# dvega68/MC33_c_library

Measured on AMD Instinct MI355X. Metric: Mvoxels/s, higher is better.
Workload: dtype f32; 1 GPU; 1024x1024x1024-point float grid cos x+cos y+cos z on h=8/1023, iso=0.0, calculate_isosurface (sweep+scan+emit), grid and outputs resident in HBM; cells=1070599167, sweep=one pass over the grid per isovalue, vertices=3903888, triangles=7795976, parallelism=single GPU

## Files before the change

### mc33_c_library_amd/build.py

```python
import os
import shutil
import subprocess
import sys

PKG = os.path.dirname(os.path.abspath(__file__))
CSRC = os.path.join(PKG, "csrc")
ROOT = os.path.dirname(PKG)
BUILD = os.path.join(PKG, "_build")

HIPCC = os.environ.get("HIPCC") or shutil.which("hipcc") or "/opt/rocm/bin/hipcc"
GCC = os.environ.get("CC") or "gcc"

HIP_FLAGS = ["-O3", "--offload-arch=gfx950", "-ffp-contract=off", "-std=c++17", "-fPIC", "-Wall", "-Wno-unused-function", "-Wno-inline-asm"]
if os.environ.get("MC33_DEV", "0") == "1":
    HIP_FLAGS.append("-DMC33_DEV")
C_FLAGS = ["-O2", "-ffp-contract=off", "-std=c11", "-fPIC", "-Wall", "-Wextra"]

VARIANTS = {
    "f32": {"hip": [], "c": []},
    "u16": {"hip": ["-DMC33_GRD_U16"], "c": ["-DINTEGER_GRD", "-DGRD_TYPE_SIZE=2"]},
    "u8": {"hip": ["-DMC33_GRD_U8"], "c": ["-DINTEGER_GRD", "-DGRD_TYPE_SIZE=1"]},
    "u32": {"hip": ["-DMC33_GRD_U32"], "c": ["-DINTEGER_GRD", "-DGRD_TYPE_SIZE=4"]},
    "f64": {"hip": ["-DMC33_GRD_F64"], "c": ["-DGRD_TYPE_SIZE=8"]},
}


def lib_path(dtype, ortho=False, nneg=False):
    return os.path.join(PKG, "libMC33_%s%s%s.so" % (dtype, "_ortho" if ortho else "", "_nneg" if nneg else ""))


NNEG_TYPES = ("f32", "u16", "u8", "u32", "f64")


def _newer(target, deps):
    if not os.path.exists(target):
        return True
    t = os.path.getmtime(target)
    return any(os.path.getmtime(d) > t for d in deps)


def _run(cmd):
    print("+ " + " ".join(cmd), flush=True)
    subprocess.check_call(cmd)


C_SOURCES = ["mc33_capi.c", "mc33_surface_io.c", "mc33_grid_io.c"]
HIP_HEADERS = ["mc33_cell.h", "mc33_lut_data.h", "mc33_rules_data.h",
               "mc33_sweep_plan.h", "mc33_records.hip.h", "mc33_sweep_pack.h", "mc33_sweep.hip.h", "mc33_tail.hip.h", "mc33_emit.hip.h", "mc33_context.hip.h", "mc33_extract.hip.h",
               "mc33_property.hip.h", "mc33_mesh.hip.h", "mc33_measure.hip.h", "mc33_topology.hip.h", "mc33_filter.hip.h", "mc33_smooth.hip.h", "mc33_cap.hip.h", "mc33_render.hip.h",
               "mc33_distance.hip.h",
               "mc33_simplify.hip.h", "mc33_clip.hip.h", "mc33_section.hip.h", "mc33_resample.hip.h", "mc33_curvature.hip.h",
               "mc33_spectrum.hip.h"]


def build(dtype, force=False, verbose_resources=False):
    os.makedirs(BUILD, exist_ok=True)
    var = VARIANTS[dtype]
    incs = [os.path.join(ROOT, "include", f) for f in ("mc33_hip.h", "marching_cubes_33.h")] + [os.path.abspath(__file__)]
    hip_src = os.path.join(CSRC, "mc33_kernels.hip")
    hip_obj = os.path.join(BUILD, "mc33_kernels_%s.o" % dtype)
    objs, relink = [hip_obj], force
    if force or _newer(hip_obj, [hip_src] + [os.path.join(CSRC, f) for f in HIP_HEADERS] + incs):
        extra = ["-Rpass-analysis=kernel-resource-usage"] if verbose_resources else []
        _run([HIPCC] + HIP_FLAGS + var["hip"] + extra + ["-c", hip_src, "-o", hip_obj])
        relink = True
    for name in C_SOURCES:
        src = os.path.join(CSRC, name)
        obj = os.path.join(BUILD, "%s_%s.o" % (os.path.splitext(name)[0], dtype))
        if force or _newer(obj, [src] + incs):
            _run([GCC] + C_FLAGS + var["c"] + ["-c", src, "-o", obj])
            relink = True
        objs.append(obj)
    out = lib_path(dtype)
    if relink or _newer(out, objs):
        _run([HIPCC, "--offload-arch=gfx950", "-shared", "-fPIC"] + objs + ["-o", out])
    oobjs, relink = [hip_obj], force
    for name in C_SOURCES:
        src = os.path.join(CSRC, name)
        obj = os.path.join(BUILD, "%s_%s_ortho.o" % (os.path.splitext(name)[0], dtype))
        if force or _newer(obj, [src] + incs):
            _run([GCC] + C_FLAGS + var["c"] + ["-DGRD_ORTHOGONAL", "-c", src, "-o", obj])
            relink = True
        oobjs.append(obj)
    oout = lib_path(dtype, ortho=True)
    if relink or _newer(oout, oobjs):
        _run([HIPCC, "--offload-arch=gfx950", "-shared", "-fPIC"] + oobjs + ["-o", oout])
    if dtype in NNEG_TYPES:
        for ortho, base in ((False, objs), (True, oobjs)):
            nobjs, relink = list(base), force
            src = os.path.join(CSRC, "mc33_capi.c")
            obj = os.path.join(BUILD, "mc33_capi_%s%s_nneg.o" % (dtype, "_ortho" if ortho else ""))
            if force or _newer(obj, [src] + incs):
                _run([GCC] + C_FLAGS + var["c"] + (["-DGRD_ORTHOGONAL"] if ortho else []) + ["-DMC33_NORMAL_NEG=1", "-c", src, "-o", obj])
                relink = True
            nobjs[1 + C_SOURCES.index("mc33_capi.c")] = obj
            nout = lib_path(dtype, ortho=ortho, nneg=True)
            if relink or _newer(nout, nobjs):
                _run([HIPCC, "--offload-arch=gfx950", "-shared", "-fPIC"] + nobjs + ["-o", nout])
    return out


def build_all(force=False):
    from concurrent.futures import ThreadPoolExecutor
    with ThreadPoolExecutor(max_workers=min(5, os.cpu_count() or 1)) as ex:
        return list(ex.map(lambda d: build(d, force), VARIANTS))


if __name__ == "__main__":
    build_all(force="--force" in sys.argv)
```

### mc33_c_library_amd/csrc/mc33_kernels.hip

```cpp
#include <hip/hip_runtime.h>

#include <cstdarg>
#include <cstddef>
#include <cstdio>
#include <cstdlib>
#include <cstring>
#include <chrono>
#include <mutex>
#include <algorithm>
#include <cmath>
#include <limits>
#include <thread>
#include <type_traits>
#include <utility>
#include <vector>

#include "../../include/mc33_hip.h"
#ifdef MC33_GRD_F64
#define MC33_REAL_DOUBLE
#endif
#if !defined(MC33_GRD_U8) && !defined(MC33_GRD_U16) && !defined(MC33_GRD_U32)
#define MC33_NAN_SAMPLES 1
#else
#define MC33_INT_SAMPLES 1
#endif
#include "mc33_cell.h"
#include "mc33_lut_data.h"
#include "mc33_rules_data.h"

using namespace mc33;

#if defined(MC33_GRD_U16)
typedef uint16_t sample_t;
#define MC33_SAMPLE_BYTES 2
#elif defined(MC33_GRD_U8)
typedef uint8_t sample_t;
#define MC33_SAMPLE_BYTES 1
#elif defined(MC33_GRD_U32)
typedef uint32_t sample_t;
#define MC33_SAMPLE_BYTES 4
#elif defined(MC33_GRD_F64)
typedef double sample_t;
#define MC33_SAMPLE_BYTES 8
#else
typedef float sample_t;
#define MC33_SAMPLE_BYTES 4
#endif

#include "mc33_sweep_plan.h"
#include "mc33_records.hip.h"
#include "mc33_sweep_pack.h"
#include "mc33_sweep.hip.h"
#include "mc33_tail.hip.h"
#include "mc33_emit.hip.h"
#include "mc33_context.hip.h"
#include "mc33_extract.hip.h"
#include "mc33_property.hip.h"
#include "mc33_mesh.hip.h"
#include "mc33_measure.hip.h"
#include "mc33_topology.hip.h"
#include "mc33_filter.hip.h"
#include "mc33_smooth.hip.h"
#include "mc33_cap.hip.h"
#include "mc33_render.hip.h"
#include "mc33_distance.hip.h"
#include "mc33_simplify.hip.h"
#include "mc33_clip.hip.h"
#include "mc33_section.hip.h"
#include "mc33_resample.hip.h"
#include "mc33_curvature.hip.h"
#include "mc33_spectrum.hip.h"
```

### mc33_c_library_amd/csrc/mc33_sweep.hip.h

```cpp

#if defined(MC33_GRD_U16)
constexpr int SWEEP_PACK = 2;
#elif defined(MC33_GRD_U8)
constexpr int SWEEP_PACK = 4;
#else
constexpr int SWEEP_PACK = 1;
#endif

template <bool V>
__global__ __launch_bounds__(256) void k_ranges(const GridView<sample_t> G, const Params P, const uint32_t nYT, const uint32_t nplanes, RangeEntry *out, RangeEntry *blocks) {
	constexpr uint32_t VS = 16u / (uint32_t)sizeof(sample_t);
	struct alignas(16) Piece { sample_t s[VS]; };
	constexpr real_t INF = std::numeric_limits<real_t>::infinity();
	__shared__ real_t s_col0[4][4][2];
	__shared__ real_t s_blk[4][RANGE_BLOCKS][2];
	const uint32_t lane = threadIdx.x & 63u, nXG = (P.nseg + 3u) / 4u, wv = (uint32_t)__builtin_amdgcn_readfirstlane((int)(threadIdx.x >> 6));
	const uint32_t xg = blockIdx.x % nXG, yt = (blockIdx.x / nXG) % nYT, pl = blockIdx.x / nXG / nYT;
	const uint32_t seg = xg * 4u + wv;
	const bool active = seg < P.nseg && pl < nplanes;
	const uint32_t xbase = seg * SEG_CELLS, y0 = yt * 63u, nrows = min(64u, P.ny + 1u - y0), xlast = min(xbase + SEG_CELLS, P.nx);
	const sample_t *base = G.p + (uint64_t)pl * G.slice + (uint64_t)y0 * G.pitch;
	const bool right = wv < 3u && seg + 1u < P.nseg;
	auto take = [&](real_t &lo, real_t &hi, sample_t s) __attribute__((always_inline)) {
		const real_t f = (real_t)s;
// ... 262 lines not shown
		whole = (e.x & MC33_PACK_GROUP) != 0u;
	}
	if (wtile >= a.ntiles) return;
	const SweepTile tile = a.tiles[wtile];
	const uint32_t yt = tile.yt, seg = tile.seg;
	const Params &P = a.P;
	bool grouped = true;
	if constexpr (R == 2) grouped = whole;
	else {
		const uint32_t t0 = wtile & ~3u;
		if (t0 + 3u >= a.ntiles) grouped = false;
		else {
			const SweepTile first = a.tiles[t0];
#pragma unroll
			for (uint32_t k = 1; k < 4; k++) {
				const SweepTile o = a.tiles[t0 + k];
				grouped = grouped && o.seg == first.seg + k && o.yt == first.yt && o.z_lo == first.z_lo && o.z_hi == first.z_hi;
			}
		}
	}
	const unsigned long long t_start = a.trace ? __builtin_amdgcn_s_memrealtime() : 0ull;
	const unsigned long long c_start = a.trace ? __builtin_amdgcn_s_memtime() : 0ull;
	if (R == 1 && a.ranges) {
		const uint32_t wme = (uint32_t)__builtin_amdgcn_readfirstlane((int)(threadIdx.x >> 6));
		const uint32_t seg0 = grouped ? seg - wme : seg, nk = grouped ? 4u : 1u, me = grouped ? wme : 0u;
		const uint32_t p0r = tile.z_lo == a.P.zs ? tile.z_lo : tile.z_lo + 1u;
		uint32_t m = 0xFFFFFFFFu;
		for (uint32_t p = p0r + lane; p <= tile.z_hi; p += 64u) {
			const RangeEntry *row = a.ranges + (((uint64_t)(p - a.G.z0) * a.sd.nYT + yt) * a.sd.nseg + seg0);
			static_for<4>([&](auto kc) __attribute__((always_inline)) {
				constexpr int k = decltype(kc)::value;
				if ((uint32_t)k < nk) {
					const RangeEntry e = row[k];
					static_for<NI>([&](auto qc) __attribute__((always_inline)) {
						constexpr int q = decltype(qc)::value;
						const real_t v = a.lane[q].iso;
						m &= ~(((e.hi < v ? 0u : 1u) | (e.lo > v ? 0u : 2u)) << (2 * NI * k + 2 * q));
					});
				}
			});
		}
#pragma unroll
		for (int dlt = 32; dlt; dlt >>= 1) m &= (uint32_t)__shfl_xor((int)m, dlt);
		m = (uint32_t)__builtin_amdgcn_readfirstlane((int)m);
		constexpr uint32_t EVEN = NI == 4 ? 0x55u : NI == 2 ? 0x5u : 0x1u, ALLQ = (1u << (2 * NI)) - 1u;
		const uint32_t one_side = (m | m >> 1);
		bool dead_any = false;
		static_for<4>([&](auto kc) __attribute__((always_inline)) {
			constexpr int k = decltype(kc)::value;
			if ((uint32_t)k < nk) dead_any = dead_any || ((one_side >> (2 * NI * k)) & EVEN) == EVEN;
		});
		const uint32_t mine = (m >> (2u * NI * me)) & ALLQ;
		dead_me = ((mine | mine >> 1) & EVEN) == EVEN;
		if (dead_any) grouped = false;
		if (dead_me) {
			if (lane == 0) {
				static_for<NI>([&](auto qc) __attribute__((always_inline)) {
					constexpr int q = decltype(qc)::value;
					const bool above = ((mine >> (2 * q)) & 2u) != 0u;
					const uint32_t hb = above ? 0xFFFFFFFFu : 0u;
					uint4 *h = a.lane[q].edge_hdr + (uint64_t)wtile * 2u * 2u;
					if (p0r != tile.z_lo) { h[0] = uint4{hb, hb, 0u, 0u}; h[1] = uint4{0u, 0u, above ? PLANE_UNIFORM1 : PLANE_UNIFORM0, 0u}; }
					if (tile.z_hi < a.z_end) { h[2] = uint4{hb, hb, 0u, 0u}; h[3] = uint4{0u, 0u, above ? PLANE_UNIFORM1 : PLANE_UNIFORM0, 0u}; }
				});
				if (NI == 1 && a.skipped) atomicAdd(a.skipped + ((mine & 2u) ? 2 : 1), 1u);
			}
		}
	}
	__shared__ uint64_t s_mail[2][4][NI][2];
	const bool from_right = grouped && (uint32_t)__builtin_amdgcn_readfirstlane((int)(threadIdx.x >> 6)) < 3u;
	const uint32_t xbase = seg * SEG_CELLS, y0 = yt * 63u;
	const uint32_t nrows = min(64u, P.ny + 1 - y0);
	const uint32_t z_lo = tile.z_lo, z_hi = tile.z_hi;
	const uint32_t pl0 = z_lo == P.zs ? z_lo : z_lo + 1u;
	const bool has_above = z_hi < a.z_end;

	const uint32_t rowbytes = a.G.pitch * (uint32_t)sizeof(sample_t);
	uint32_t xo[LPR];
#pragma unroll
	for (int k = 0; k < LPR; k++)
		xo[k] = S == 1 ? min(xbase + 64u * k + lane, P.nx) * (uint32_t)sizeof(sample_t)
		               : min(xbase + (256u / LPR) * k + (uint32_t)S * lane, P.nx & ~(uint32_t)(S - 1)) * (uint32_t)sizeof(sample_t);
	uint64_t valid[4];
	{
		uint64_t vstd[4];
		valid_masks(xbase, P.nx, vstd);
		from_standard<S>(vstd, valid);
	}
	const bool rowvalid = lane < 63u && y0 + lane < P.ny;
	const uint32_t xh = min(lane, nrows - 1) * rowbytes + min(xbase + SEG_CELLS, P.nx) * (uint32_t)sizeof(sample_t);

	constexpr bool PREV_LDS = NI >= 4;
	__shared__ uint64_t s_prev[PREV_LDS ? NI : 1][4][PREV_LDS ? 256 : 1];
	__shared__ uint64_t s_prevz[PREV_LDS ? NI : 1][2][4];
	__shared__ uint32_t s_prevh[PREV_LDS ? NI : 1][PREV_LDS ? 256 : 1];
	constexpr bool DEFER = NI == 1;
	__shared__ typename std::conditional<DEFER, SweepLog, uint32_t>::type s_log[DEFER ? 4 : 1];
	uint32_t log_np = 0, log_ns = 0, log_edge = LOG_NONE;
	uint32_t pend_chunk[NI];
	unsigned long long pend_sum[NI];
#pragma unroll
	for (int q = 0; q < NI; q++) { pend_chunk[q] = 0u; pend_sum[q] = 0ull; }
	const uint32_t wv = (uint32_t)__builtin_amdgcn_readfirstlane((int)(threadIdx.x >> 6));
	uint64_t cur[NI][4], prev[PREV_LDS ? 1 : NI][4];
	uint64_t c64[NI][4];
	uint32_t cur_h[NI], prev_h[PREV_LDS ? 1 : NI];
	uint64_t cur_zc[NI], prev_zc[PREV_LDS ? 1 : NI], zcacc[NI];
	uint64_t cur_z[NI], prev_z[PREV_LDS ? 1 : NI], zacc[NI];
	constexpr bool ZMIN_REG = !(sizeof(real_t) == 8 && NI >= 4);
	real_t zmin[NI];
	uint64_t zeq[NI];
	bool cur_written[NI], prev_written[NI];
	real_t iso[NI];
#pragma unroll
	for (int q = 0; q < NI; q++) {
#pragma unroll
		for (int k = 0; k < 4; k++) {
			if constexpr (PREV_LDS) s_prev[q][k][threadIdx.x] = 0; else prev[q][k] = 0;
			c64[q][k] = 0;
		}
		cur_h[q] = 0; cur_z[q] = zacc[q] = 0; cur_zc[q] = zcacc[q] = 0;
		if constexpr (PREV_LDS) { s_prevz[q][0][wv] = 0; s_prevz[q][1][wv] = 0; s_prevh[q][threadIdx.x] = 0; } else { prev_z[q] = 0; prev_zc[q] = 0; prev_h[q] = 0; }
		cur_written[q] = prev_written[q] = false; zmin[q] = 1; zeq[q] = 0;
		iso[q] = a.lane[q].iso;
	}

	const uint32_t NB = (nrows + (uint32_t)RB - 1u) / (uint32_t)RB;
	const uint32_t T = dead_me ? 0u : (z_hi - pl0 + 1u) * NB;
	const uint32_t tile_bytes = dead_me ? 0u : nrows * rowbytes;
#ifndef MC33_SWEEP_AUX
#if defined(MC33_GRD_U16) || defined(MC33_GRD_U8)
#define MC33_SWEEP_AUX 0
#else
#define MC33_SWEEP_AUX 2
#endif
#endif
#if defined(MC33_GRD_U16)
#define MC33_LOAD(rs, vo, so) ((float)(uint16_t)__builtin_amdgcn_raw_buffer_load_b16(rs, vo, so, MC33_SWEEP_AUX))
#elif defined(MC33_GRD_U8)
#define MC33_LOAD(rs, vo, so) ((float)(uint8_t)__builtin_amdgcn_raw_buffer_load_b8(rs, vo, so, MC33_SWEEP_AUX))
#elif defined(MC33_GRD_U32)
#define MC33_LOAD(rs, vo, so) ((float)(uint32_t)__builtin_amdgcn_raw_buffer_load_b32(rs, vo, so, MC33_SWEEP_AUX))
#elif defined(MC33_GRD_F64)
#define MC33_LOAD(rs, vo, so) (__builtin_bit_cast(double, __builtin_amdgcn_raw_buffer_load_b64(rs, vo, so, MC33_SWEEP_AUX)))
#else
#define MC33_LOAD(rs, vo, so) (__uint_as_float(__builtin_amdgcn_raw_buffer_load_b32(rs, vo, so, MC33_SWEEP_AUX)))
#endif
	typedef typename std::conditional<S == 1, real_t, uint32_t>::type raw_t;
	constexpr bool BS = BLOCKS;
	static_assert(!BLOCKS || (MC33_BLOCK_SKIP && R == 2 && NI == 1 && S == 1), "blocks are left out by the float single-isovalue sweep with a live list");
	auto block_word = [&](uint32_t p) __attribute__((always_inline)) -> uint64_t {
		if constexpr (BS) {
			if (a.blockw) {
				const unsigned long long w = a.blockw[((uint64_t)(min(p, z_hi) - a.G.z0) * a.sd.nYT + yt) * a.sd.nseg + seg];
				return u64((uint32_t)__builtin_amdgcn_readfirstlane((int)(uint32_t)w), (uint32_t)__builtin_amdgcn_readfirstlane((int)(uint32_t)(w >> 32)));
			}
		}
		return 0ull;
	};
	uint64_t bwi = block_word(pl0), bwi_n = block_word(pl0 + 1u), bwp = bwi, bwp_n = bwi_n;
	auto issue = [&](raw_t (&d)[16], real_t &hv, uint32_t p, uint32_t bi) __attribute__((always_inline)) {
		const sample_t *base = a.G.p + (uint64_t)(p - a.G.z0) * a.G.slice + (uint64_t)y0 * a.G.pitch;
		const __amdgpu_buffer_rsrc_t rs = __builtin_amdgcn_make_buffer_rsrc((void *)base, 0, tile_bytes, 0x00020000);
		const uint32_t r = bi * (uint32_t)RB;
		uint32_t codes = 0u, hcode = 0u;
		if constexpr (BS) { codes = (uint32_t)(bwi >> (8u * (bi >> 2))) & 0xFFu; hcode = (uint32_t)(bwi >> (32u + 2u * (bi >> 2))) & 3u; }
#pragma unroll
		for (int rr = 0; rr < RB; rr++) {
			const uint32_t so = min(r + rr, nrows - 1) * rowbytes;
#pragma unroll
			for (int k = 0; k < LPR; k++) {
				if constexpr (BS) {
					const bool dk = ((codes >> (2 * k)) & 3u) != 0u;
					d[rr * LPR + k] = MC33_LOAD(rs, dk ? 0xFFFFFFF0u : xo[k], dk ? 0u : so);
				} else
				if constexpr (S == 1) d[rr * LPR + k] = MC33_LOAD(rs, xo[k], so);
				else d[rr * LPR + k] = __builtin_amdgcn_raw_buffer_load_b32(rs, xo[k], so, MC33_SWEEP_AUX);
			}
		}
		if constexpr (NI == 1 && sizeof(real_t) == 4) {
			const bool wanted = ((lane / (uint32_t)RB) == bi) & !from_right & !(MC33_DEBUG_BITS(a) & 64u) & (hcode == 0u);
			if (wanted) hv = MC33_LOAD(rs, xh, 0u);
		} else
		hv = MC33_LOAD(rs, ((lane / (uint32_t)RB) == bi && !from_right && !(MC33_DEBUG_BITS(a) & 64u)) ? xh : 0xFFFFFFF0u, 0u);
	};
	auto sample = [&](const raw_t (&dd)[16], int rr, int k) -> real_t {
		if constexpr (S == 1) return dd[rr * 4 + k];
		else if constexpr (S == 2) return (real_t)((dd[rr * 2 + (k >> 1)] >> (16 * (k & 1))) & 0xFFFFu);
		else return (real_t)((dd[rr] >> (8 * k)) & 0xFFu);
	};

	auto raw_sample = [&](const raw_t (&dd)[16], int rr, int k) -> uint32_t {
		if constexpr (S == 2) return ((uint32_t)dd[rr * 2 + (k >> 1)] >> (16 * (k & 1))) & 0xFFFFu;
		else if constexpr (S == 4) return ((uint32_t)dd[rr] >> (8 * k)) & 0xFFu;
		else return 0u;
	};
	auto log_flush = [&]() __attribute__((always_inline)) {
		if constexpr (DEFER) {
			SweepLog &G = s_log[wv];
			const SweepLane &L0 = a.lane[0];
			const uint32_t ln = fresh_lane();
			__builtin_amdgcn_fence(__ATOMIC_ACQ_REL, "wavefront");
			for (uint32_t k = 0; k < log_np; k++) {
				const uint64_t slot = readlane64(G.plane_slot[k], 0);
				__builtin_amdgcn_raw_buffer_store_b32(G.plane[k][ln], record_rsrc(L0.slice_compact + slot * 64u, 256u), ln * 4u, 0u, 0);
				if (ln == 0) L0.plane_fmt[slot] = (uint8_t)PLANE_COMPACT;
			}
			{
				const bool mine = ln < log_ns;
				const uint32_t e = mine ? ln : 0u;
				const uint32_t *w = G.hdr[e];
				const uint64_t slot = G.hdr_slot[e];
				if (mine) {
					uint32_t *h = (uint32_t *)(L0.slice_hdr + slot);
					*(uint4 *)h = uint4{w[0], w[1], w[2], w[3]};
					*(uint4 *)(h + 4) = uint4{w[4], w[5], w[6], w[7]};
					*(uint2 *)(h + 8) = uint2{w[8], w[9]};
				}
				const uint32_t chunk = mine ? (uint32_t)(slot / SLOT_CHUNK) : 0xFFFFFFFFu;
				const uint32_t cells = mine ? w[5] : 0u, batches = mine ? w[10] : 0u;
				uint32_t sum_c = cells, sum_b = batches;
#pragma unroll 1
				for (uint32_t dlt = 1; dlt < log_ns; dlt++) {
					const uint32_t c2 = __shfl_down(chunk, dlt), v2 = __shfl_down(cells, dlt), b2 = __shfl_down(batches, dlt);
					const bool same = c2 == chunk && ln + dlt < 64u;
					sum_c += same ? v2 : 0u; sum_b += same ? b2 : 0u;
				}
				const uint32_t before = __shfl_up(chunk, 1);
				if (mine && (ln == 0u || before != chunk)) atomicAdd(L0.slot_part + chunk, (unsigned long long)sum_b << 32 | sum_c);
			}
			if (log_edge != LOG_NONE) {
				if (log_edge == PLANE_COMPACT) __builtin_amdgcn_raw_buffer_store_b32(G.edge[ln], record_rsrc(L0.edge_bits + (uint64_t)wtile * 2u * 128u, 2048u), ln * 4u, 0u, 0);
				if (ln == 0) {
					const uint32_t *e = G.edge_hdr;
					L0.edge_hdr[(uint64_t)wtile * 2u * 2u] = uint4{e[0], e[1], e[2], e[3]};
					L0.edge_hdr[(uint64_t)wtile * 2u * 2u + 1u] = uint4{e[4], e[5], e[6], e[7]};
				}
			}
			__builtin_amdgcn_fence(__ATOMIC_ACQ_REL, "wavefront");
			log_np = 0; log_ns = 0; log_edge = LOG_NONE;
		}
	};
	auto log_plane = [&](uint64_t slot, const uint64_t (&w)[4], uint32_t ln) __attribute__((always_inline)) {
		if constexpr (DEFER) {
			uint32_t desc;
			if (encode_plane<S>(w, desc)) {
				if (log_np == LOG_PLANES) log_flush();
				SweepLog &G = s_log[wv];
				G.plane[log_np][ln] = desc;
				if (ln == 0) G.plane_slot[log_np] = slot;
				log_np++;
			} else {
				store_plane_raw<S>(a.lane[0].slice_bits + slot * 128u, w, ln);
				if (ln == 0) a.lane[0].plane_fmt[slot] = (uint8_t)PLANE_RAW;
			}
		}
	};
	auto log_header = [&](uint64_t slot, uint64_t bp, uint64_t bc, uint64_t zrows, uint64_t zcols, const uint64_t (&act)[4], uint32_t ln) __attribute__((always_inline)) {
		if constexpr (DEFER) {
			uint32_t ncell = __popcll(act[0]) + __popcll(act[1]) + __popcll(act[2]) + __popcll(act[3]);
#pragma unroll
			for (int dlt = 32; dlt; dlt >>= 1) ncell += __shfl_xor(ncell, dlt);
			if (log_ns == LOG_SLICES) log_flush();
			if (ln == 0) {
				SweepLog &G = s_log[wv];
				uint32_t *w = G.hdr[log_ns];
				w[0] = a.lane[0].epoch << 2 | SLICE_VALID | (zrows ? SLICE_HAS_ISO : 0u);
				w[1] = (uint32_t)bp; w[2] = (uint32_t)(bp >> 32); w[3] = (uint32_t)bc; w[4] = (uint32_t)(bc >> 32); w[5] = ncell;
				w[6] = (uint32_t)zrows; w[7] = (uint32_t)(zrows >> 32); w[8] = (uint32_t)zcols; w[9] = (uint32_t)(zcols >> 32);
				w[10] = (ncell + 63u) >> 6;
				G.hdr_slot[log_ns] = slot;
			}
			log_ns++;
		}
	};
	real_t halo = 0;
	auto process = [&](const raw_t (&dd)[16], const real_t &hv, uint32_t p, uint32_t bi) __attribute__((always_inline)) {
		const uint32_t r = bi * (uint32_t)RB;
		uint32_t codes = 0u;
		if constexpr (BS) {
			constexpr real_t INF = std::numeric_limits<real_t>::infinity();
			codes = (uint32_t)(bwp >> (8u * (bi >> 2))) & 0xFFu;
			const uint32_t hcode = (uint32_t)(bwp >> (32u + 2u * (bi >> 2))) & 3u;
			const real_t hsub = hcode == 1u ? -INF : INF;
			halo = (lane / (uint32_t)RB) == bi ? (hcode ? hsub : hv) : halo;
		} else
		halo = (lane / (uint32_t)RB) == bi ? hv : halo;
		unrolled_for<RB, (S >= 4)>([&](auto rc) __attribute__((always_inline)) {
			const int rr = rc;
			real_t f[4];
#pragma unroll
			for (int k = 0; k < 4; k++) f[k] = sample(dd, rr, k);
			if constexpr (BS) {
				constexpr real_t INF = std::numeric_limits<real_t>::infinity();
#pragma unroll
				for (int k = 0; k < 4; k++) {
					const uint32_t ck = (codes >> (2 * k)) & 3u;
					f[k] = ck ? (ck == 1u ? -INF : INF) : f[k];
				}
			}
			uint64_t bwq[NI][4];
			static_for<NI>([&](auto qc) __attribute__((always_inline)) {
				constexpr int q = decltype(qc)::value;
				uint64_t bw[4];
#pragma unroll
				for (int k = 0; k < 4; k++) {
					uint64_t bb;
					if constexpr (ZM == 0) {
						const real_t d = iso[q] - f[k];
						bb = __ballot(sign_of(d) != 0);
#ifdef MC33_NAN_SAMPLES
						bb ^= __ballot(d != d);
#endif
						if constexpr (ZMIN_REG) zmin[q] = real_min(zmin[q], real_abs(d));
						else zeq[q] |= __ballot(d == 0);
					} else if constexpr (S >= 2) {
						const uint32_t ri = raw_sample(dd, rr, k);
						bb = __ballot((int32_t)ri > a.lane[q].iso_gt);
						if constexpr (ZM == 1) zeq[q] |= __ballot(ri == a.lane[q].iso_eq);
					} else {
						bb = __ballot(f[k] > iso[q]);
						if constexpr (ZM == 1) zeq[q] |= __ballot(f[k] == iso[q]);
					}
					bw[k] = bb;
				}
				const uint32_t rowsel = (uint32_t)__builtin_amdgcn_readfirstlane((int)(r + (uint32_t)rr));
				if constexpr (NI >= 2) {
#pragma unroll
					for (int k = 0; k < 4; k++) bwq[q][k] = bw[k];
				} else {
					uint64_t &w0 = c64[q][0], &w1 = c64[q][1], &w2 = c64[q][2], &w3 = c64[q][3];
					uint64_t saved;
					asm volatile(
					    "s_mov_b64 %4, exec\n\t"
					    "s_lshl_b64 exec, 1, %9\n\t"
					    "v_mov_b64 %0, %5\n\tv_mov_b64 %1, %6\n\tv_mov_b64 %2, %7\n\tv_mov_b64 %3, %8\n\t"
					    "s_mov_b64 exec, %4"
					    : "+v"(w0), "+v"(w1), "+v"(w2), "+v"(w3), "=&s"(saved)
					    : "s"(bw[0]), "s"(bw[1]), "s"(bw[2]), "s"(bw[3]), "s"(rowsel)
					    : "scc");
				}
			});
			if constexpr (NI >= 2) {
				static_for<NI / 2>([&](auto hc) __attribute__((always_inline)) {
					constexpr int q0 = 2 * decltype(hc)::value;
					const uint32_t rowsel = (uint32_t)__builtin_amdgcn_readfirstlane((int)(r + (uint32_t)rr));
					uint64_t &w0 = c64[q0][0], &w1 = c64[q0][1], &w2 = c64[q0][2], &w3 = c64[q0][3];
					uint64_t &w4 = c64[q0 + 1][0], &w5 = c64[q0 + 1][1], &w6 = c64[q0 + 1][2], &w7 = c64[q0 + 1][3];
					const uint64_t b0 = bwq[q0][0], b1 = bwq[q0][1], b2 = bwq[q0][2], b3 = bwq[q0][3];
					const uint64_t b4 = bwq[q0 + 1][0], b5 = bwq[q0 + 1][1], b6 = bwq[q0 + 1][2], b7 = bwq[q0 + 1][3];
					uint64_t saved;
					asm volatile(
					    "s_mov_b64 %8, exec\n\t"
					    "s_lshl_b64 exec, 1, %17\n\t"
					    "v_mov_b64 %0, %9\n\tv_mov_b64 %1, %10\n\tv_mov_b64 %2, %11\n\tv_mov_b64 %3, %12\n\t"
					    "v_mov_b64 %4, %13\n\tv_mov_b64 %5, %14\n\tv_mov_b64 %6, %15\n\tv_mov_b64 %7, %16\n\t"
					    "s_mov_b64 exec, %8"
					    : "+v"(w0), "+v"(w1), "+v"(w2), "+v"(w3), "+v"(w4), "+v"(w5), "+v"(w6), "+v"(w7), "=&s"(saved)
					    : "s"(b0), "s"(b1), "s"(b2), "s"(b3), "s"(b4), "s"(b5), "s"(b6), "s"(b7), "s"(rowsel)
					    : "scc");
				});
			}
		});
		if constexpr (ZM != 2)
			static_for<NI>([&](auto qc) __attribute__((always_inline)) {
				constexpr int q = decltype(qc)::value;
				const uint64_t zb = (ZM == 0 && ZMIN_REG) ? __ballot(zmin[q] == 0) : zeq[q];
				if (zb) { zacc[q] |= ((1ull << RB) - 1ull) << r; zcacc[q] |= zb; }
				zmin[q] = 1; zeq[q] = 0;
			});
		if (bi != NB - 1) return;
		const uint32_t lp = NI >= 2 ? fresh_lane() : lane;
		const uint32_t tid = NI >= 2 ? wv * 64u + lp : threadIdx.x;
		const uint32_t par = (p - pl0) & 1u;
		if (grouped) {
			static_for<NI>([&](auto qc) __attribute__((always_inline)) {
				constexpr int q = decltype(qc)::value;
				const uint64_t hb = __ballot(((uint32_t)c64[q][0] & 1u) != 0u);
				if (lp == 0) {
					s_mail[par][wv][q][0] = hb;
					s_mail[par][wv][q][1] = (ZM != 2 && (zcacc[q] & 1ull)) ? zacc[q] : 0ull;
				}
			});
			asm volatile("s_waitcnt lgkmcnt(0)\n\ts_barrier" ::: "memory");
		}
		static_for<NI>([&](auto qc) __attribute__((always_inline)) {
			constexpr int q = decltype(qc)::value;
			const SweepLane &L = a.lane[q];
#pragma unroll
			for (int k = 0; k < 4; k++) { cur[q][k] = c64[q][k]; c64[q][k] = 0; }
			if (from_right) {
				const uint64_t nb_bits = s_mail[par][wv + 1u][q][0], nb_zero = ZM != 2 ? s_mail[par][wv + 1u][q][1] : 0ull;
				cur_h[q] = (uint32_t)((nb_bits >> lp) & 1ull);
				const uint64_t zh = nb_zero & (nrows >= 64u ? ~0ull : ((1ull << nrows) - 1ull));
				cur_z[q] = zacc[q] | zh;
				cur_zc[q] = zh ? ~0ull : zcacc[q];
				zacc[q] = zcacc[q] = 0;
			} else {
				const real_t dh = iso[q] - halo;
				cur_h[q] = sign_of(dh);
#ifdef MC33_NAN_SAMPLES
				cur_h[q] ^= (uint32_t)(dh != dh);
#endif
				const uint64_t zh = __ballot(lp < nrows && dh == 0);
				cur_z[q] = zacc[q] | zh;
				cur_zc[q] = zh ? ~0ull : zcacc[q];
				zacc[q] = zcacc[q] = 0;
			}
			auto leave_edge = [&](uint32_t which) __attribute__((always_inline)) {
				uint32_t fmt = PLANE_RAW;
				uint4 *rec = L.edge_bits + ((uint64_t)wtile * 2u + which) * 128u;
				const uint64_t w_or = cur[q][0] | cur[q][1] | cur[q][2] | cur[q][3], w_and = cur[q][0] & cur[q][1] & cur[q][2] & cur[q][3];
				const bool all0 = __ballot(w_or != 0ull) == 0ull, all1 = __ballot(w_and != ~0ull) == 0ull;
				bool deferred = false;
				if (all0 || all1) { fmt = all0 ? PLANE_UNIFORM0 : PLANE_UNIFORM1; deferred = DEFER && which == 0u && !MC33_DEBUG_BITS(a); }
				else if (DEFER && which == 0u && !MC33_DEBUG_BITS(a)) {
					uint32_t desc;
					if (encode_plane<S>(cur[q], desc)) {
						if constexpr (DEFER) s_log[wv].edge[lp] = desc;
						fmt = PLANE_COMPACT; deferred = true;
					} else store_plane_raw<S>(rec, cur[q], lp);
				}
				else fmt = store_plane_record<S>(rec, (uint32_t *)rec, cur[q], lp);
				const uint64_t bh = __ballot(cur_h[q] != 0);
				if (deferred) {
					if constexpr (DEFER) {
						if (lp == 0) {
							uint32_t *e = s_log[wv].edge_hdr;
							e[0] = (uint32_t)bh; e[1] = (uint32_t)(bh >> 32); e[2] = (uint32_t)cur_z[q]; e[3] = (uint32_t)(cur_z[q] >> 32);
							e[4] = (uint32_t)cur_zc[q]; e[5] = (uint32_t)(cur_zc[q] >> 32); e[6] = fmt; e[7] = 0u;
						}
						log_edge = fmt;
					}
				} else
				if (lp == 0 && !(MC33_DEBUG_BITS(a) & 4096u)) {
					L.edge_hdr[((uint64_t)wtile * 2u + which) * 2u] = uint4{(uint32_t)bh, (uint32_t)(bh >> 32), (uint32_t)cur_z[q], (uint32_t)(cur_z[q] >> 32)};
					L.edge_hdr[((uint64_t)wtile * 2u + which) * 2u + 1u] = uint4{(uint32_t)cur_zc[q], (uint32_t)(cur_zc[q] >> 32), fmt, 0u};
				}
			};
			if (MC33_DEBUG_BITS(a) & 2u) {
			} else {
				if (p == pl0 && pl0 != z_lo && !(MC33_DEBUG_BITS(a) & (256u | 1024u))) leave_edge(0);
				if (p > pl0 && !(MC33_DEBUG_BITS(a) & 512u)) {
					uint64_t act[4], pq[4];
#pragma unroll
					for (int k = 0; k < 4; k++) {
						if constexpr (PREV_LDS) pq[k] = s_prev[q][k][tid]; else pq[k] = prev[q][k];
					}
					uint32_t ph;
					if constexpr (PREV_LDS) ph = s_prevh[q][tid]; else ph = prev_h[q];
					active_cells<S>(pq, cur[q], ph, cur_h[q], valid, rowvalid, act);
					if (__ballot((act[0] | act[1] | act[2] | act[3]) != 0ull) && !(MC33_DEBUG_BITS(a) & 16u)) {
						uint64_t pz, pzc;
						if constexpr (PREV_LDS) { pz = readlane64(s_prevz[q][0][wv], 0); pzc = readlane64(s_prevz[q][1][wv], 0); }
						else { pz = prev_z[q]; pzc = prev_zc[q]; }
						if (DEFER && !MC33_DEBUG_BITS(a)) {
							const uint64_t slot = slice_slot(p - 1 - P.zs, yt, seg, a.sd), slot_up = slice_slot(p - P.zs, yt, seg, a.sd);
							if (!prev_written[q]) log_plane(slot, pq, lp);
							log_plane(slot_up, cur[q], lp);
							log_header(slot, __ballot(ph != 0), __ballot(cur_h[q] != 0), pz | cur_z[q], pzc | cur_zc[q], act, lp);
						} else
						hand_over_slice<S>(L, slice_slot(p - 1 - P.zs, yt, seg, a.sd), slice_slot(p - P.zs, yt, seg, a.sd), pq, cur[q],
						                   !prev_written[q], true, __ballot(ph != 0), __ballot(cur_h[q] != 0), pz | cur_z[q], pzc | cur_zc[q], act, lp,
						                   MC33_DEBUG_BITS(a), NI >= 2 ? &pend_chunk[q] : nullptr, NI >= 2 ? &pend_sum[q] : nullptr);
						cur_written[q] = true;
					}
				}
				if (p == z_hi && has_above && !(MC33_DEBUG_BITS(a) & (256u | 2048u))) leave_edge(1);
			}
#pragma unroll
			for (int k = 0; k < 4; k++) {
				if constexpr (PREV_LDS) s_prev[q][k][tid] = cur[q][k]; else prev[q][k] = cur[q][k];
			}
			if constexpr (PREV_LDS) s_prevh[q][tid] = cur_h[q]; else prev_h[q] = cur_h[q];
			if constexpr (PREV_LDS) { s_prevz[q][0][wv] = cur_z[q]; s_prevz[q][1][wv] = cur_zc[q]; } else { prev_z[q] = cur_z[q]; prev_zc[q] = cur_zc[q]; }
			prev_written[q] = cur_written[q];
			cur_written[q] = false;
			if constexpr (NI >= 2) __builtin_amdgcn_sched_barrier(0);
		});
	};

	raw_t dA[16], dB[16];
	real_t hA = 0, hB = 0;
	uint32_t ip = pl0, ib = 0, pp = pl0, pb = 0;
#define MC33_ADV(p_, b_, w_, wn_) do { if (++(b_) == NB) { (b_) = 0; ++(p_); if constexpr (BS) { (w_) = (wn_); (wn_) = block_word((p_) + 1u); } } } while (0)
#define MC33_ADV_ISSUE() do { if (ip != z_hi || ib + 1 != NB) MC33_ADV(ip, ib, bwi, bwi_n); } while (0)
	issue(dA, hA, ip, ib); MC33_ADV_ISSUE();
#ifdef MC33_DEV
	if (MC33_DEBUG_BITS(a) & 16384u) {
		auto drop = [&](const raw_t (&dd)[16], const real_t &hv) __attribute__((always_inline)) {
#pragma unroll
			for (int k = 0; k < 16; k++) asm volatile("" ::"v"(dd[k]));
			asm volatile("" ::"v"(hv));
		};
		for (uint32_t t = 0; t < T; t += 2) {
			issue(dB, hB, ip, ib); MC33_ADV_ISSUE();
			drop(dA, hA);
			issue(dA, hA, ip, ib); MC33_ADV_ISSUE();
			drop(dB, hB);
		}
		return;
	}
#endif
	for (uint32_t t = 0; t < T; t += 2) {
		issue(dB, hB, ip, ib); MC33_ADV_ISSUE();
		process(dA, hA, pp, pb); MC33_ADV(pp, pb, bwp, bwp_n);
		issue(dA, hA, ip, ib); MC33_ADV_ISSUE();
		if (t + 1 < T) { process(dB, hB, pp, pb); MC33_ADV(pp, pb, bwp, bwp_n); }
	}
	log_flush();
	if constexpr (NI >= 2) {
#pragma unroll
		for (int q = 0; q < NI; q++)
			if (pend_sum[q] && lane == 0) atomicAdd(a.lane[q].slot_part + pend_chunk[q], pend_sum[q]);
	}
	if (a.trace && lane == 0) {
		unsigned long long *tr = a.trace + 4ull * (blockIdx.x * 4u + wv);
		tr[0] = t_start; tr[1] = __builtin_amdgcn_s_memrealtime(); tr[2] = c_start; tr[3] = __builtin_amdgcn_s_memtime();
	}
#undef MC33_ADV_ISSUE
#undef MC33_ADV
#undef MC33_LOAD
}
template <int S, int NI, int ZM = 0>
__global__ __launch_bounds__(256) __attribute__((amdgpu_waves_per_eu(3))) void k_sweep(const SweepArgs a) {
	sweep_tile<S, NI, ZM, 1>(a);
}
template <int S, int NI, int ZM = 0>
__global__ __launch_bounds__(256) __attribute__((amdgpu_waves_per_eu(3))) void k_sweep_live(const SweepArgs a) {
	sweep_tile<S, NI, ZM, 2>(a);
}
template <int ZM = 0>
__global__ __launch_bounds__(256) __attribute__((amdgpu_waves_per_eu(3))) void k_sweep_live_blocks(const SweepArgs a) {
	if constexpr (MC33_BLOCK_SKIP) sweep_tile<1, 1, ZM, 2, true>(a);
}
template <int S, int NI, int ZM = 0>
__global__ __launch_bounds__(256) __attribute__((amdgpu_waves_per_eu(3))) void k_sweep_all(const SweepArgs a) {
	sweep_tile<S, NI, ZM, 0>(a);
}

__global__ __launch_bounds__(256) void k_boundary(const SweepArgs a, const TileBoundary *bounds, uint32_t nbounds) {
	const SweepLane &L = a.lane[blockIdx.y];
	const uint32_t lane = threadIdx.x & 63u;
	const uint32_t bi = blockIdx.x * 4u + (uint32_t)__builtin_amdgcn_readfirstlane((int)(threadIdx.x >> 6));
	if (bi >= nbounds) return;
	const TileBoundary b = bounds[bi];
	const Params &P = a.P;
	const uint32_t seg = b.seg;
	const uint64_t rp = (uint64_t)b.below * 2u + 1u, rc = (uint64_t)b.above * 2u;
	const uint4 hp = L.edge_hdr[rp * 2u], hc = L.edge_hdr[rc * 2u], zp = L.edge_hdr[rp * 2u + 1u], zc = L.edge_hdr[rc * 2u + 1u];
	if (zp.z >= PLANE_UNIFORM0 && zp.z == zc.z) {
		const uint32_t side = zp.z == PLANE_UNIFORM1 ? 0xFFFFFFFFu : 0u;
		if (hp.x == side && hp.y == side && hc.x == side && hc.y == side) return;
	}
	const uint4 p0 = L.edge_bits[rp * 128u + lane], p1 = L.edge_bits[rp * 128u + 64u + lane];
	const uint4 c0 = L.edge_bits[rc * 128u + lane], c1 = L.edge_bits[rc * 128u + 64u + lane];
	const uint32_t dp = ((const uint32_t *)(L.edge_bits + rp * 128u))[lane], dc = ((const uint32_t *)(L.edge_bits + rc * 128u))[lane];
	uint64_t prev[4] = {u64(p0.x, p0.y), u64(p0.z, p0.w), u64(p1.x, p1.y), u64(p1.z, p1.w)};
	uint64_t cur[4] = {u64(c0.x, c0.y), u64(c0.z, c0.w), u64(c1.x, c1.y), u64(c1.z, c1.w)};
	if (zp.z == PLANE_COMPACT) decode_row(dp, prev);
	if (zc.z == PLANE_COMPACT) decode_row(dc, cur);
	if (zp.z >= PLANE_UNIFORM0) { prev[0] = prev[1] = prev[2] = prev[3] = zp.z == PLANE_UNIFORM1 ? ~0ull : 0ull; }
	if (zc.z >= PLANE_UNIFORM0) { cur[0] = cur[1] = cur[2] = cur[3] = zc.z == PLANE_UNIFORM1 ? ~0ull : 0ull; }
	const uint64_t bp = u64(hp.x, hp.y), bc = u64(hc.x, hc.y);
	uint64_t valid[4], act[4];
	valid_masks(seg * SEG_CELLS, P.nx, valid);
	const bool rowvalid = lane < 63u && b.yt * 63u + lane < P.ny;
	active_cells(prev, cur, (uint32_t)((bp >> lane) & 1ull), (uint32_t)((bc >> lane) & 1ull), valid, rowvalid, act);
	if (__ballot((act[0] | act[1] | act[2] | act[3]) != 0ull))
		hand_over_slice<1>(L, slice_slot(b.z - P.zs, b.yt, seg, a.sd), slice_slot(b.z + 1u - P.zs, b.yt, seg, a.sd), prev, cur,
		                true, true, bp, bc, u64(hp.z, hp.w) | u64(hc.z, hc.w), u64(zp.x, zp.y) | u64(zc.x, zc.y), act, lane);
}
```

Baseline: 2.154 million Mvoxels/s.

## Skip constant blocks in sweep by iterating only live blocks per plane

In the block-summary (BS) sweep path, the loop no longer visits every row block of every plane with dummy loads for constant blocks. It now walks a bitmask of live (non-constant) 16-row by 64-column blocks, issuing loads and sign ballots only for those and seeding constant blocks' bit words and halo directly from the block codes. The block word is also read through a constant address space pointer so it becomes a scalar load instead of a vector load followed by readfirstlane. This is meant to cut load and ALU work on planes that are mostly far from the isosurface, at the cost of a more complex, data-dependent control loop with its own double-buffered issue and process steps.

```diff
diff --git a/mc33_c_library_amd/build.py b/mc33_c_library_amd/build.py
--- a/mc33_c_library_amd/build.py
+++ b/mc33_c_library_amd/build.py
@@ -46,7 +46,7 @@
 
 C_SOURCES = ["mc33_capi.c", "mc33_surface_io.c", "mc33_grid_io.c"]
 HIP_HEADERS = ["mc33_cell.h", "mc33_lut_data.h", "mc33_rules_data.h",
-               "mc33_sweep_plan.h", "mc33_records.hip.h", "mc33_sweep_pack.h", "mc33_sweep.hip.h", "mc33_tail.hip.h", "mc33_emit.hip.h", "mc33_context.hip.h", "mc33_extract.hip.h",
+               "mc33_sweep_plan.h", "mc33_sweep_blocks.h", "mc33_records.hip.h", "mc33_sweep_pack.h", "mc33_sweep.hip.h", "mc33_tail.hip.h", "mc33_emit.hip.h", "mc33_context.hip.h", "mc33_extract.hip.h",
                "mc33_property.hip.h", "mc33_mesh.hip.h", "mc33_measure.hip.h", "mc33_topology.hip.h", "mc33_filter.hip.h", "mc33_smooth.hip.h", "mc33_cap.hip.h", "mc33_render.hip.h",
                "mc33_distance.hip.h",
                "mc33_simplify.hip.h", "mc33_clip.hip.h", "mc33_section.hip.h", "mc33_resample.hip.h", "mc33_curvature.hip.h",
diff --git a/mc33_c_library_amd/csrc/mc33_kernels.hip b/mc33_c_library_amd/csrc/mc33_kernels.hip
--- a/mc33_c_library_amd/csrc/mc33_kernels.hip
+++ b/mc33_c_library_amd/csrc/mc33_kernels.hip
@@ -48,6 +48,7 @@
 #endif
 
 #include "mc33_sweep_plan.h"
+#include "mc33_sweep_blocks.h"
 #include "mc33_records.hip.h"
 #include "mc33_sweep_pack.h"
 #include "mc33_sweep.hip.h"
diff --git a/mc33_c_library_amd/csrc/mc33_sweep.hip.h b/mc33_c_library_amd/csrc/mc33_sweep.hip.h
--- a/mc33_c_library_amd/csrc/mc33_sweep.hip.h
+++ b/mc33_c_library_amd/csrc/mc33_sweep.hip.h
@@ -438,34 +438,27 @@
 	auto block_word = [&](uint32_t p) __attribute__((always_inline)) -> uint64_t {
 		if constexpr (BS) {
 			if (a.blockw) {
-				const unsigned long long w = a.blockw[((uint64_t)(min(p, z_hi) - a.G.z0) * a.sd.nYT + yt) * a.sd.nseg + seg];
-				return u64((uint32_t)__builtin_amdgcn_readfirstlane((int)(uint32_t)w), (uint32_t)__builtin_amdgcn_readfirstlane((int)(uint32_t)(w >> 32)));
+				typedef const __attribute__((address_space(4))) unsigned long long *const_words_t;
+				return ((const_words_t)(uintptr_t)a.blockw)[((uint64_t)(min(p, z_hi) - a.G.z0) * a.sd.nYT + yt) * a.sd.nseg + seg];
 			}
 		}
 		return 0ull;
 	};
-	uint64_t bwi = block_word(pl0), bwi_n = block_word(pl0 + 1u), bwp = bwi, bwp_n = bwi_n;
 	auto issue = [&](raw_t (&d)[16], real_t &hv, uint32_t p, uint32_t bi) __attribute__((always_inline)) {
 		const sample_t *base = a.G.p + (uint64_t)(p - a.G.z0) * a.G.slice + (uint64_t)y0 * a.G.pitch;
 		const __amdgpu_buffer_rsrc_t rs = __builtin_amdgcn_make_buffer_rsrc((void *)base, 0, tile_bytes, 0x00020000);
 		const uint32_t r = bi * (uint32_t)RB;
-		uint32_t codes = 0u, hcode = 0u;
-		if constexpr (BS) { codes = (uint32_t)(bwi >> (8u * (bi >> 2))) & 0xFFu; hcode = (uint32_t)(bwi >> (32u + 2u * (bi >> 2))) & 3u; }
 #pragma unroll
 		for (int rr = 0; rr < RB; rr++) {
 			const uint32_t so = min(r + rr, nrows - 1) * rowbytes;
 #pragma unroll
 			for (int k = 0; k < LPR; k++) {
-				if constexpr (BS) {
-					const bool dk = ((codes >> (2 * k)) & 3u) != 0u;
-					d[rr * LPR + k] = MC33_LOAD(rs, dk ? 0xFFFFFFF0u : xo[k], dk ? 0u : so);
-				} else
 				if constexpr (S == 1) d[rr * LPR + k] = MC33_LOAD(rs, xo[k], so);
 				else d[rr * LPR + k] = __builtin_amdgcn_raw_buffer_load_b32(rs, xo[k], so, MC33_SWEEP_AUX);
 			}
 		}
 		if constexpr (NI == 1 && sizeof(real_t) == 4) {
-			const bool wanted = ((lane / (uint32_t)RB) == bi) & !from_right & !(MC33_DEBUG_BITS(a) & 64u) & (hcode == 0u);
+			const bool wanted = ((lane / (uint32_t)RB) == bi) & !from_right & !(MC33_DEBUG_BITS(a) & 64u);
 			if (wanted) hv = MC33_LOAD(rs, xh, 0u);
 		} else
 		hv = MC33_LOAD(rs, ((lane / (uint32_t)RB) == bi && !from_right && !(MC33_DEBUG_BITS(a) & 64u)) ? xh : 0xFFFFFFF0u, 0u);
@@ -563,28 +556,13 @@
 	real_t halo = 0;
 	auto process = [&](const raw_t (&dd)[16], const real_t &hv, uint32_t p, uint32_t bi) __attribute__((always_inline)) {
 		const uint32_t r = bi * (uint32_t)RB;
-		uint32_t codes = 0u;
-		if constexpr (BS) {
-			constexpr real_t INF = std::numeric_limits<real_t>::infinity();
-			codes = (uint32_t)(bwp >> (8u * (bi >> 2))) & 0xFFu;
-			const uint32_t hcode = (uint32_t)(bwp >> (32u + 2u * (bi >> 2))) & 3u;
-			const real_t hsub = hcode == 1u ? -INF : INF;
-			halo = (lane / (uint32_t)RB) == bi ? (hcode ? hsub : hv) : halo;
-		} else
+		if constexpr (!BS) {
 		halo = (lane / (uint32_t)RB) == bi ? hv : halo;
 		unrolled_for<RB, (S >= 4)>([&](auto rc) __attribute__((always_inline)) {
 			const int rr = rc;
 			real_t f[4];
 #pragma unroll
 			for (int k = 0; k < 4; k++) f[k] = sample(dd, rr, k);
-			if constexpr (BS) {
-				constexpr real_t INF = std::numeric_limits<real_t>::infinity();
-#pragma unroll
-				for (int k = 0; k < 4; k++) {
-					const uint32_t ck = (codes >> (2 * k)) & 3u;
-					f[k] = ck ? (ck == 1u ? -INF : INF) : f[k];
-				}
-			}
 			uint64_t bwq[NI][4];
 			static_for<NI>([&](auto qc) __attribute__((always_inline)) {
 				constexpr int q = decltype(qc)::value;
@@ -655,6 +633,7 @@
 				if (zb) { zacc[q] |= ((1ull << RB) - 1ull) << r; zcacc[q] |= zb; }
 				zmin[q] = 1; zeq[q] = 0;
 			});
+		}
 		if (bi != NB - 1) return;
 		const uint32_t lp = NI >= 2 ? fresh_lane() : lane;
 		const uint32_t tid = NI >= 2 ? wv * 64u + lp : threadIdx.x;
@@ -768,9 +747,122 @@
 
 	raw_t dA[16], dB[16];
 	real_t hA = 0, hB = 0;
+	if constexpr (BS) {
+		const uint32_t nrg = (NB + 3u) >> 2;
+		const bool own_halo = !from_right;
+		const uint32_t lg = lane >> 4;
+		const bool lane_in = lane < NB * 4u;
+		const uint64_t rows_in = NB >= 16u ? ~0ull : (1ull << (4u * NB)) - 1ull;
+		const uint32_t xl = xbase + lane, so_last = (nrows - 1u) * rowbytes;
+		uint64_t bwi = block_word(pl0), bwi_n = block_word(pl0 + 1u), bwp = bwi, bwp_n = bwi_n;
+		uint32_t ip = pl0, pp = pl0;
+		uint32_t rem_i = sweep_live_mask(bwi, nrg, own_halo), rem_p = rem_i;
+		auto issue_next = [&](raw_t (&d)[16], real_t &hv) __attribute__((always_inline)) -> bool {
+			while (rem_i == 0u && ip < z_hi) {
+				++ip; bwi = bwi_n; bwi_n = block_word(ip + 1u);
+				rem_i = sweep_live_mask(bwi, nrg, own_halo);
+			}
+			const bool there = rem_i != 0u;
+			const uint32_t j = there ? sweep_next_block(rem_i, 0u) : 0u;
+			rem_i &= rem_i - 1u;
+			const uint32_t g = j >> 2, k = j & 3u;
+			const sample_t *base = a.G.p + (uint64_t)(ip - a.G.z0) * a.G.slice + (uint64_t)y0 * a.G.pitch;
+			const __amdgpu_buffer_rsrc_t rs = __builtin_amdgcn_make_buffer_rsrc((void *)base, 0, there ? tile_bytes : 0u, 0x00020000);
+			const uint32_t vo = min(xl + 64u * k, P.nx) * (uint32_t)sizeof(sample_t);
+			uint32_t so = 16u * g * rowbytes;
+#pragma unroll
+			for (int rr = 0; rr < 16; rr++) {
+				d[rr] = MC33_LOAD(rs, vo, so);
+				so = min(so + rowbytes, so_last);
+			}
+			const bool wanted = (lg == g) & lane_in & (k == 3u) & own_halo & there & !(MC33_DEBUG_BITS(a) & 64u) & (sweep_halo_code(bwi, g) == 0u);
+			if (wanted) hv = MC33_LOAD(rs, xh, 0u);
+			return there;
+		};
+		auto plane_start = [&]() __attribute__((always_inline)) {
+#pragma unroll
+			for (int k = 0; k < 4; k++) c64[0][k] = lane_in ? sweep_const_word(bwp, lg, (uint32_t)k) : 0ull;
+			halo = lane_in ? __uint_as_float(sweep_const_halo_bits(bwp, lg)) : 0.0f;
+		};
+		auto process_next = [&](const raw_t (&dd)[16], const real_t &hv, bool have) __attribute__((always_inline)) -> bool {
+			if (have) {
+				const uint32_t j = sweep_next_block(rem_p, 0u);
+				rem_p &= rem_p - 1u;
+				const uint32_t g = j >> 2, k = j & 3u;
+				uint64_t row = 0;
+#pragma unroll
+				for (int rr = 0; rr < 16; rr++) {
+					const real_t d = iso[0] - dd[rr];
+					uint64_t bb = __ballot(sign_of(d) != 0);
+#ifdef MC33_NAN_SAMPLES
+					bb ^= __ballot(d != d);
+#endif
+					zmin[0] = real_min(zmin[0], real_abs(d));
+					const uint32_t rowsel = (uint32_t)__builtin_amdgcn_readfirstlane((int)(16u * g + (uint32_t)rr));
+					uint64_t saved;
+					asm volatile(
+					    "s_mov_b64 %1, exec\n\t"
+					    "s_lshl_b64 exec, 1, %3\n\t"
+					    "v_mov_b64 %0, %2\n\t"
+					    "s_mov_b64 exec, %1"
+					    : "+v"(row), "=&s"(saved)
+					    : "s"(bb), "s"(rowsel)
+					    : "scc");
+				}
+				const bool mine = (lg == g) & lane_in;
+#pragma unroll
+				for (int kk = 0; kk < 4; kk++) c64[0][kk] = (mine & (k == (uint32_t)kk)) ? row : c64[0][kk];
+				if (k == 3u && sweep_halo_code(bwp, g) == 0u) halo = mine ? hv : halo;
+				const uint64_t zb = __ballot(zmin[0] == 0);
+				if (zb) { zacc[0] |= (0xFFFFull << (16u * g)) & rows_in; zcacc[0] |= zb; }
+				zmin[0] = 1;
+			}
+			while (rem_p == 0u) {
+				process(dd, hv, pp, NB - 1u);
+				if (pp == z_hi) {
+					__builtin_amdgcn_s_waitcnt(0x0F70);
+					return true;
+				}
+				++pp; bwp = bwp_n; bwp_n = block_word(pp + 1u);
+				rem_p = sweep_live_mask(bwp, nrg, own_halo);
+				plane_start();
+			}
+			return false;
+		};
+		if (!dead_me) {
+			plane_start();
+			bool have = rem_p != 0u;
+#ifdef MC33_DEV
+			if (MC33_DEBUG_BITS(a) & 16384u) {
+				auto drop = [&](const raw_t (&dd)[16], const real_t &hv) __attribute__((always_inline)) {
+#pragma unroll
+					for (int k = 0; k < 16; k++) asm volatile("" ::"v"(dd[k]));
+					asm volatile("" ::"v"(hv));
+				};
+				bool more = issue_next(dA, hA);
+				while (more) {
+					more = issue_next(dB, hB);
+					drop(dA, hA);
+					if (!more) break;
+					more = issue_next(dA, hA);
+					drop(dB, hB);
+				}
+				return;
+			}
+#endif
+			if (have) issue_next(dA, hA);
+			for (;;) {
+				issue_next(dB, hB);
+				if (process_next(dA, hA, have)) break;
+				issue_next(dA, hA);
+				if (process_next(dB, hB, true)) break;
+				have = true;
+			}
+		}
+	} else {
 	uint32_t ip = pl0, ib = 0, pp = pl0, pb = 0;
-#define MC33_ADV(p_, b_, w_, wn_) do { if (++(b_) == NB) { (b_) = 0; ++(p_); if constexpr (BS) { (w_) = (wn_); (wn_) = block_word((p_) + 1u); } } } while (0)
-#define MC33_ADV_ISSUE() do { if (ip != z_hi || ib + 1 != NB) MC33_ADV(ip, ib, bwi, bwi_n); } while (0)
+#define MC33_ADV(p_, b_) do { if (++(b_) == NB) { (b_) = 0; ++(p_); } } while (0)
+#define MC33_ADV_ISSUE() do { if (ip != z_hi || ib + 1 != NB) MC33_ADV(ip, ib); } while (0)
 	issue(dA, hA, ip, ib); MC33_ADV_ISSUE();
 #ifdef MC33_DEV
 	if (MC33_DEBUG_BITS(a) & 16384u) {
@@ -790,9 +882,10 @@
 #endif
 	for (uint32_t t = 0; t < T; t += 2) {
 		issue(dB, hB, ip, ib); MC33_ADV_ISSUE();
-		process(dA, hA, pp, pb); MC33_ADV(pp, pb, bwp, bwp_n);
+		process(dA, hA, pp, pb); MC33_ADV(pp, pb);
 		issue(dA, hA, ip, ib); MC33_ADV_ISSUE();
-		if (t + 1 < T) { process(dB, hB, pp, pb); MC33_ADV(pp, pb, bwp, bwp_n); }
+		if (t + 1 < T) { process(dB, hB, pp, pb); MC33_ADV(pp, pb); }
+	}
 	}
 	log_flush();
 	if constexpr (NI >= 2) {
diff --git a/mc33_c_library_amd/csrc/mc33_sweep_blocks.h b/mc33_c_library_amd/csrc/mc33_sweep_blocks.h
--- /dev/null
+++ b/mc33_c_library_amd/csrc/mc33_sweep_blocks.h
@@ -0,0 +1,46 @@
+#ifndef MC33_SWEEP_BLOCKS_H
+#define MC33_SWEEP_BLOCKS_H
+#include <stdint.h>
+
+#if defined(__HIPCC__) || defined(__CUDACC__)
+#define MC33_BLOCKS_FN __host__ __device__ static inline
+#else
+#define MC33_BLOCKS_FN static inline
+#endif
+
+constexpr uint32_t SWEEP_BLOCK_NONE = 16u;
+
+MC33_BLOCKS_FN uint32_t sweep_block_code(uint64_t word, uint32_t g, uint32_t k) { return (uint32_t)(word >> (8u * g + 2u * k)) & 3u; }
+MC33_BLOCKS_FN uint32_t sweep_halo_code(uint64_t word, uint32_t g) { return (uint32_t)(word >> (32u + 2u * g)) & 3u; }
+
+MC33_BLOCKS_FN uint32_t sweep_live_mask(uint64_t word, uint32_t row_groups, bool own_halo) {
+	const uint32_t lo = (uint32_t)word, hi = (uint32_t)(word >> 32);
+	uint32_t e = ~(lo | lo >> 1) & 0x55555555u;
+	e = (e | e >> 1) & 0x33333333u;
+	e = (e | e >> 2) & 0x0F0F0F0Fu;
+	e = (e | e >> 4) & 0x00FF00FFu;
+	e = (e | e >> 8) & 0x0000FFFFu;
+	if (own_halo) {
+		const uint32_t h = ~(hi | hi >> 1) & 0x55u;
+		e |= (h & 1u) << 3 | (h & 4u) << 5 | (h & 16u) << 7 | (h & 64u) << 9;
+	}
+	return e & ((1u << (4u * row_groups)) - 1u);
+}
+
+MC33_BLOCKS_FN uint32_t sweep_next_block(uint32_t mask, uint32_t j) {
+	const uint32_t m = j < 16u ? (mask & 0xFFFFu) >> j << j : 0u;
+#if defined(__HIP_DEVICE_COMPILE__)
+	return m ? (uint32_t)__builtin_ctz(m) : SWEEP_BLOCK_NONE;
+#else
+	for (uint32_t b = j; b < 16u; b++)
+		if ((m >> b) & 1u) return b;
+	return SWEEP_BLOCK_NONE;
+#endif
+}
+
+MC33_BLOCKS_FN uint64_t sweep_const_word(uint64_t word, uint32_t g, uint32_t k) { return sweep_block_code(word, g, k) == 2u ? ~0ull : 0ull; }
+MC33_BLOCKS_FN uint32_t sweep_const_halo_bits(uint64_t word, uint32_t g) {
+	const uint32_t c = sweep_halo_code(word, g);
+	return c == 0u ? 0u : c == 1u ? 0xFF800000u : 0x7F800000u;
+}
+#endif
```

Result: faster. 2.546 million Mvoxels/s (median of 6 runs) (+18.2%).
